# Superjie13/StereoTracking

Measured on AMD Instinct MI355X. Metric: stereo frame-pairs/sec @1280x720 D=192, higher is better.
Workload: dtype f32; 1 GPU; configs[1]: batch=8 synthetic 1280x720 stereo pairs per GPU, D=192, full YOLOX-s two-branch backbone+PAFPN+head, cost volume at 1/4 res (48 levels) + 2 3x3 aggregation convs + soft-argmin, decode+NMS, per-box depth; global_batch=8, inflight_contexts=4, distinct_input_batches=4, gpu_max_hw_queues=4, hip_force_dev_kernarg=1, parallelism=single process, no process group (no collective in the step), collectives_issued=0, tuning_plan=configs/tuning/mi355x.json, max_det=1000, detections_overflow=False

## Files before the change

include/stereotrack.h:

```cpp
#ifndef STEREOTRACK_H_
#define STEREOTRACK_H_

#include <stddef.h>
#include <stdint.h>

#ifdef __cplusplus
extern "C" {
#endif

#define ST_VERSION 430

enum {
  ST_OK = 0,
  ST_ERR_INVALID = -1,
  ST_ERR_HIP = -2,
  ST_ERR_STATE = -3,
  ST_ERR_WORKSPACE = -4,
  ST_ERR_NOTFOUND = -5
};

typedef void* st_stream_t;

int st_version(void);
const char* st_last_error(void);

typedef struct StConvDesc {
  const float* in_dev;
  int N, Hi, Wi, Cin, in_ld, in_off;
  const float* wgt_dev;
  const float* bias_dev;
  int Cout, KH, KW, stride, pad;
  float* out1_dev;
  int out1_ld, out1_off, split;
  float* out2_dev;
  int out2_ld, out2_off;
  float* up_dev;
  int up_ld, up_off;
  const float* res_dev;
  int res_ld, res_off;
  float post_scale;
  int act;
  const float* wgt_wino_dev;
} StConvDesc;

int st_conv2d_nhwc(const StConvDesc* d, st_stream_t stream);
int st_conv2d_nhwc_variant(const StConvDesc* d, st_stream_t stream, int variant);
size_t st_wino_packed_floats(int Cout, int Cin);
int st_wino_pack_weights(const float* packed_wgt_host, int Cout, int Cin, float* out_host);

int st_conv1x1_chain(const StConvDesc* a, const StConvDesc* b, st_stream_t stream);
size_t st_front_frag_floats(int Cout, int Cin);
int st_front_pack_frags(const float* packed_wgt_host, int Cout, int Cin, float* out_host);
int st_conv3x3s2_csp_front(const StConvDesc* a, const StConvDesc* ms, const StConvDesc* c1, const float* frag_ms_dev,
                           const float* frag_c1_dev, st_stream_t stream);
size_t st_csp_tail_frag_floats(void);
int st_csp_tail_pack_frags(const float* packed_wgt_host, float* out_host);
int st_conv3x3_csp_tail(const StConvDesc* conv2, const StConvDesc* fin, const float* frag_fin_dev, st_stream_t stream);
size_t st_conv_packed_floats(int Cout, int Cin, int KH, int KW);
int st_conv_pack_weights(const float* w, const float* conv_bias,
                         const float* bn_gamma, const float* bn_beta,
                         const float* bn_mean, const float* bn_var,
                         double bn_eps, int Cout, int Cin, int KH, int KW,
                         float* wgt_out, float* bias_out);

int st_focus_pack(const float* img_nchw_dev, int N, int C, int H, int W,
                  float* out_nhwc_dev, st_stream_t stream);

size_t st_stem_packed_floats(int Cout);
int st_stem_pack_weights(const float* w, const float* conv_bias,
                         const float* bn_gamma, const float* bn_beta,
                         const float* bn_mean, const float* bn_var,
                         double bn_eps, int Cout, int used_planes, float* wgt_out, float* bias_out);
int st_stem_focus_conv(const float* img_nchw_dev, int N, int H, int W, int used_planes, const float* wgt_dev,
                       const float* bias_dev, int Cout, float* out_nhwc_dev, int out_ld, int out_off,
                       int act , st_stream_t stream);
int st_stem_focus_conv_u8(const unsigned char* const* frames_u8_dev_ptrs_host, int N, int h, int w, int H, int W,
                          float pad_value, const float* wgt_dev, const float* bias_dev, int Cout, float* out_dev,
                          int out_ld, int out_off, int act, st_stream_t stream);

int st_pack_raw_inputs(const unsigned char* img_u8_dev, const unsigned short* disp_u16_dev, int N, int h, int w,
                       int H, int W, float img_pad, float* img_out_dev, float* disp_postp_out_dev,
// ... 292 lines not shown
```

stereotracking_amd/_lib.py:

```python
import ctypes as C
import os

import torch

_HERE = os.path.dirname(os.path.abspath(__file__))
LIB_PATH = os.path.join(_HERE, 'lib', 'libstereotrack_hip.so')

ST_OK = 0
_ERR_NAMES = {-1: 'ST_ERR_INVALID', -2: 'ST_ERR_HIP', -3: 'ST_ERR_STATE', -4: 'ST_ERR_WORKSPACE',
              -5: 'ST_ERR_NOTFOUND'}


class StError(RuntimeError):
    """A libstereotrack_hip call returned a non-zero status."""


class StConvDesc(C.Structure):
    _fields_ = [
        ('in_dev', C.c_void_p),
        ('N', C.c_int), ('Hi', C.c_int), ('Wi', C.c_int), ('Cin', C.c_int), ('in_ld', C.c_int), ('in_off', C.c_int),
        ('wgt_dev', C.c_void_p), ('bias_dev', C.c_void_p),
        ('Cout', C.c_int), ('KH', C.c_int), ('KW', C.c_int), ('stride', C.c_int), ('pad', C.c_int),
        ('out1_dev', C.c_void_p), ('out1_ld', C.c_int), ('out1_off', C.c_int), ('split', C.c_int),
        ('out2_dev', C.c_void_p), ('out2_ld', C.c_int), ('out2_off', C.c_int),
# ... 55 lines not shown
        ('score_thr', C.c_float), ('iou_thr', C.c_float), ('max_det', C.c_int),
        ('scale_x', C.c_float), ('scale_y', C.c_float), ('pad_left', C.c_float), ('pad_top', C.c_float),
        ('ori_w', C.c_float), ('ori_h', C.c_float), ('nms_mask_rows', C.c_int), ('num_classes', C.c_int),
        ('single_label', C.c_int),
    ]


_vp, _i, _f, _sz = C.c_void_p, C.c_int, C.c_float, C.c_size_t
_PROTOS = {
    'st_version': (C.c_int, []),
    'st_head_row_floats': (_i, [_i]),
    'st_png_unfilter': (_i, [_vp, _i, _i, _i, _vp]),
    'st_stem_focus_conv_u8': (_i, [_vp, _i, _i, _i, _i, _i, _f, _vp, _vp, _i, _vp, _i, _i, _i, _vp]),
    'st_detector_forward_raw': (_i, [_vp, _vp, _i, _i, _f, _vp, _vp, _sz, _vp, _vp]),
    'st_detector_forward_phase0_raw': (_i, [_vp, _vp, _vp, _i, _i, _f, _vp, _sz, _vp]),
    'st_pack_raw_frames': (_i, [_vp, _i, _i, _i, _i, _i, _f, _vp, _vp]),
    'st_resize_planes': (_i, [_vp, _i, _i, _i, _i, _vp, _i, _i, _i, _i, _vp]),
    'st_detector_set_split': (_i, [_vp, _i]),
    'st_split_instances_available': (_i, []),
    'st_volume_agg3d': (_i, [_vp, _vp, _i, _i, _i, _i, _vp, _f, _i, _vp]),
    'st_last_error': (C.c_char_p, []),
    'st_conv2d_nhwc': (_i, [C.POINTER(StConvDesc), _vp]),
    'st_conv2d_nhwc_variant': (_i, [C.POINTER(StConvDesc), _vp, _i]),
    'st_conv1x1_chain': (_i, [C.POINTER(StConvDesc), C.POINTER(StConvDesc), _vp]),
    'st_front_frag_floats': (_sz, [_i, _i]),
    'st_front_pack_frags': (_i, [_vp, _i, _i, _vp]),
    'st_conv3x3s2_csp_front': (_i, [C.POINTER(StConvDesc), C.POINTER(StConvDesc), C.POINTER(StConvDesc), _vp, _vp, _vp]),
    'st_csp_tail_frag_floats': (_sz, []),
    'st_csp_tail_pack_frags': (_i, [_vp, _vp]),
    'st_conv3x3_csp_tail': (_i, [C.POINTER(StConvDesc), C.POINTER(StConvDesc), _vp, _vp]),
    'st_conv_packed_floats': (_sz, [_i, _i, _i, _i]),
    'st_wino_packed_floats': (_sz, [_i, _i]),
    'st_wino_pack_weights': (_i, [_vp, _i, _i, _vp]),
    'st_conv_pack_weights': (_i, [_vp, _vp, _vp, _vp, _vp, _vp, C.c_double, _i, _i, _i, _i, _vp, _vp]),
    'st_focus_pack': (_i, [_vp, _i, _i, _i, _i, _vp, _vp]),
    'st_stem_packed_floats': (_sz, [_i]),
    'st_stem_pack_weights': (_i, [_vp, _vp, _vp, _vp, _vp, _vp, C.c_double, _i, _i, _vp, _vp]),
    'st_stem_focus_conv': (_i, [_vp, _i, _i, _i, _i, _vp, _vp, _i, _vp, _i, _i, _i, _vp]),
    'st_pack_raw_inputs': (_i, [_vp, _vp, _i, _i, _i, _i, _i, _f, _vp, _vp, _vp, _vp]),
    'st_spp_pool': (_i, [_vp, _i, _i, _i, _i, _i, _i, _vp, _i, _i, _vp]),
    'st_detector_create': (_i, [C.POINTER(StDetectorConfig), C.POINTER(_vp)]),
    'st_detector_destroy': (_i, [_vp]),
    'st_detector_num_params': (_i, [_vp]),
    'st_detector_param_info': (_i, [_vp, _i, C.c_char_p, _i, C.POINTER(C.c_int64), C.POINTER(_i)]),
    'st_detector_set_param': (_i, [_vp, C.c_char_p, _vp, C.c_int64]),
    'st_detector_finalize': (_i, [_vp]),
    'st_detector_workspace_bytes': (_sz, [_vp]),
    'st_detector_head_floats': (_sz, [_vp]),
    'st_detector_num_levels': (_i, [_vp]),
    'st_detector_level_info': (_i, [_vp, _i, C.POINTER(_i), C.POINTER(_i), C.POINTER(_i), C.POINTER(_sz)]),
    'st_detector_forward': (_i, [_vp, _vp, _vp, _vp, _sz, _vp, _vp]),
    'st_detector_forward_phase': (_i, [_vp, _i, _vp, _vp, _vp, _vp, _sz, _vp, _vp]),
    'st_detector_macs': (C.c_double, [_vp]),
    'st_detector_set_timing': (_i, [_vp, _i]),
    'st_detector_num_ops': (_i, [_vp]),
    'st_detector_op_times': (_i, [_vp, _i, _vp, _vp, _vp, _vp, _vp]),
    'st_detector_autotune': (_i, [_vp, _vp, _sz, _vp, _vp, _i]),
    'st_conv_variant_name': (C.c_char_p, [_i]),
    'st_conv_variant_signature': (C.c_char_p, [_i]),
    'st_detector_get_tuning': (_i, [_vp, _vp, _i]),
    'st_detector_set_tuning': (_i, [_vp, _vp, _i]),
    'st_detector_op_desc': (_i, [_vp, _i, C.c_char_p, _i]),
    'st_detector_tap': (_i, [_vp, C.c_char_p, _vp, C.POINTER(_vp), C.POINTER(_i), C.POINTER(_i),
                             C.POINTER(_i), C.POINTER(_i), C.POINTER(_i)]),
    'st_decode_nms_workspace_bytes': (_sz, [C.POINTER(StDecodeDesc)]),
    'st_lapjv_extended': (_i, [_vp, _i, _i, C.c_double, _vp, _vp]),
# ... 91 lines not shown
```

stereotracking_amd/csrc/conv_igemm.hip:

```cpp
#include <algorithm>

#include <type_traits>

#include "st_common.h"

namespace st {

typedef float f32x16 __attribute__((ext_vector_type(16)));
typedef float f32x4 __attribute__((ext_vector_type(4)));
typedef unsigned int u32x4 __attribute__((ext_vector_type(4)));

struct ConvKArgs {
  const float* in;
  const float* wgt;
  const float* bias;
  float* out1;
  float* out2;
  float* up;
  const float* res;
  int Hi, Wi, Cin, in_ld, in_off;
  int Ho, Wo, HoWo, Cout;
  int KH, KW, stride, pad;
  int K, Kpad, M;
  unsigned in_bytes, wgt_bytes;
// ... 656 lines not shown
  return id >= 0 && id < kNumVariants && round_up(cout, 32) % kVariants[id].bn == 0;
}
const char* conv_variant_name(int id) {
  static const char* names[] = {"128x128", "128x64w2", "128x32w2", "64x64", "64x32w2",
                                "128x64", "128x32", "64x128", "256x64", "64x64w1", "64x32w1", "32x64w1",
                                "128x128dma", "64x64dma", "64x128dma", "128x32dma", "128x64dma",
                                "128x128dmab", "64x64dmab", "256x128dma", "256x128dmab", "256x128",
                                "128x128ws", "64x64ws", "64x128ws", "128x32ws", "128x64ws", "128x128ws2",
                                "64x128ws2", "128x128ws4"};
  return id >= 0 && id < kNumVariants ? names[id] : "-";
}

const char* conv_variant_signature(int id) {
  static const char* sigs[] = {"2, 2, 2, 2, 2, 1, 0", "2, 2, 2, 1, 2, 1, 0", "2, 1, 2, 1, 2, 1, 0",
                               "1, 1, 2, 2, 2, 1, 0", "1, 1, 2, 1, 2, 1, 0", "1, 2, 4, 1, 2, 1, 0",
                               "1, 1, 4, 1, 2, 1, 0", "1, 2, 2, 2, 2, 1, 0", "2, 2, 4, 1, 2, 1, 0",
                               "2, 2, 1, 1, 1, 1, 0", "2, 1, 1, 1, 1, 1, 0", "1, 2, 1, 1, 1, 1, 0",
                               "2, 2, 2, 2, 2, 1, 1", "1, 1, 2, 2, 2, 1, 1", "1, 2, 2, 2, 2, 1, 1",
                               "1, 1, 4, 1, 2, 1, 1", "1, 2, 4, 1, 2, 1, 1", "2, 2, 2, 2, 2, 0, 1",
                               "1, 1, 2, 2, 2, 0, 1", "2, 2, 4, 2, 2, 1, 1", "2, 2, 4, 2, 2, 0, 1",
                               "2, 2, 4, 2, 2, 1, 0", "ws 2, 2, 2, 2", "ws 1, 1, 2, 2", "ws 1, 2, 2, 2",
                               "ws 1, 1, 4, 1", "ws 1, 2, 4, 1", "ws 2, 2, 2, 2, 2", "ws 1, 2, 2, 2, 2",
                               "ws 2, 2, 2, 2, 4"};
  return id >= 0 && id < kNumVariants ? sigs[id] : "";
}

bool pw_conv_applicable(const StConvDesc& d);
int pw_conv_launch(const StConvDesc& d, hipStream_t stream, const StConvDesc* chain);
int pwr_conv_launch(const StConvDesc& d, hipStream_t stream, const StConvDesc* chain);
bool pwr_chain_applicable(const StConvDesc& d, const StConvDesc& c);
bool dc_conv_applicable(const StConvDesc& d);
int dc_conv_launch(const StConvDesc& d, hipStream_t stream);
bool wino_conv_applicable(const StConvDesc& d);
int wino_conv_launch(const StConvDesc& d, hipStream_t stream, bool narrow);
int wino_persist_launch(const StConvDesc& d, hipStream_t stream);

int conv2d_launch(const StConvDesc& d, hipStream_t stream, int force_variant, int* picked_variant) {
  ST_REQUIRE(d.in_dev && d.wgt_dev && d.bias_dev && d.out1_dev, "conv: null pointer");
  if (force_variant == 41) {
    if (picked_variant) *picked_variant = 41;
    return pw_conv_launch(d, stream, nullptr);
  }
  if (force_variant == 46) {
    if (picked_variant) *picked_variant = 46;
    return pwr_conv_launch(d, stream, nullptr);
  }
  if (force_variant == 42) {
    if (picked_variant) *picked_variant = 42;
    return dc_conv_launch(d, stream);
  }
  if (force_variant == 43 || force_variant == 44) {
    if (picked_variant) *picked_variant = force_variant;
    return wino_conv_launch(d, stream, force_variant == 44);
  }
#ifdef ST_ABLATION
  if (force_variant == 57) {
    if (picked_variant) *picked_variant = 57;
    return wino_persist_launch(d, stream);
  }
#endif
  ST_REQUIRE(d.Cin % 4 == 0 && d.in_ld % 4 == 0 && d.in_off % 4 == 0,
             "conv: Cin/in_ld/in_off must be multiples of 4 (got %d/%d/%d)", d.Cin, d.in_ld,
             d.in_off);
  ST_REQUIRE(d.N > 0 && d.Hi > 0 && d.Wi > 0 && d.Cout > 0 && d.KH > 0 && d.KW > 0 &&
                 d.stride > 0 && d.pad >= 0,
             "conv: bad geometry");
  ST_REQUIRE(d.in_off + d.Cin <= d.in_ld, "conv: input channel slice exceeds in_ld");
  const int Ho = (d.Hi + 2 * d.pad - d.KH) / d.stride + 1;
  const int Wo = (d.Wi + 2 * d.pad - d.KW) / d.stride + 1;
  ST_REQUIRE(Ho > 0 && Wo > 0, "conv: empty output");
  const int split = (d.out2_dev ? d.split : d.Cout);
  ST_REQUIRE(split >= 0 && split <= d.Cout, "conv: bad split");
  ST_REQUIRE(d.out1_off + split <= d.out1_ld, "conv: out1 slice exceeds out1_ld");
  if (d.out2_dev)
    ST_REQUIRE(d.out2_off + (d.Cout - split) <= d.out2_ld, "conv: out2 slice exceeds out2_ld");
  if (d.up_dev) ST_REQUIRE(d.up_off + d.Cout <= d.up_ld, "conv: up slice exceeds up_ld");
  if (d.res_dev) ST_REQUIRE(d.res_off + d.Cout <= d.res_ld, "conv: res slice exceeds res_ld");
  const long long M_ll = (long long)d.N * Ho * Wo;
  ST_REQUIRE(M_ll * (long long)std::max(std::max(d.out1_ld, d.out2_ld), d.res_dev ? d.res_ld : 1) < (1ll << 31) &&
                 (long long)d.N * d.Hi * d.Wi * d.in_ld < (1ll << 29) &&
                 d.KH * d.KW <= 32 &&
                 (!d.up_dev || 4 * M_ll * d.up_ld < (1ll << 31)),
             "conv: tensor exceeds 2^31 elements");
  ST_REQUIRE((long long)d.N * d.Hi * d.Wi < (1ll << 31) && M_ll < (1ll << 31),
             "conv: pixel count exceeds int32");

// ... 116 lines not shown
```

stereotracking_amd/csrc/detector.cpp:

```cpp
#include <algorithm>
#include <cmath>
#include <cstring>
#include <map>
#include <memory>
#include <vector>

#include "st_common.h"

namespace st {

int conv2d_launch(const StConvDesc& d, hipStream_t stream, int force_variant, int* picked_variant);
bool pw_conv_applicable(const StConvDesc& d);
bool pw_chain_applicable(const StConvDesc& d, const StConvDesc& c);
bool dc_conv_applicable(const StConvDesc& d);
bool wino_conv_applicable(const StConvDesc& d);
bool wino_shape_ok(int Cin, int Cout);
bool wino_group_applicable(const StConvDesc* d, int n);
int wino_group_launch(const StConvDesc* d, int n, hipStream_t stream);
size_t wino_packed_floats(int Cout, int Cin);
int wino_pack_weights(const float* packed, int Cout, int Cin, float* out);
int pw_conv_launch(const StConvDesc& d, hipStream_t stream, const StConvDesc* chain);
bool pwr_conv_applicable(const StConvDesc& d);
bool pwr_chain_applicable(const StConvDesc& d, const StConvDesc& c);
int pwr_conv_launch(const StConvDesc& d, hipStream_t stream, const StConvDesc* chain);
// ... 995 lines not shown
        ms = std::min(ms, t);
      }
      if (rc != ST_OK) break;
      if (best_v < 0 || ms < best * 0.97f) { best = ms; best_v = v; }
    }
    saved[oi].tuned = best_v;
  }
  det->force_variant = -1;
  det->ops = saved;
  det->timing = was_timing;
  (void)hipEventDestroy(e0);
  (void)hipEventDestroy(e1);
  return rc;
}

extern "C" int st_split_instances_available(void) {
#ifdef ST_ABLATION
  return 1;
#else
  return 0;
#endif
}

extern "C" int st_detector_set_split(StDetector* det, int allow) {
  if (!det) return set_error(ST_ERR_INVALID, "st_detector_set_split: null detector");
  if (allow != 0 && !st_split_instances_available())
    return set_error(ST_ERR_INVALID, "st_detector_set_split: the split-operand (bf16x3) instances are not part of the product "
                                     "library (parked in the tools build: make ABLATION=1, ST_LIBRARY=<that library>)");
  det->allow_split = allow == 1 ? 0x3F : (allow & 0x3F);
  return ST_OK;
}

extern "C" const char* st_conv_variant_name(int id) {
  return id == 56 ? "wino32tail" : id == 47 ? "headpred" : id == 46 ? "pwres" : id == 45 ? "front3x3s2" : id == 40 ? "stem6x6s2" : id == 41 ? "pw128" : id == 42 ? "dc4x32" : id == 43 ? "wino2x2" : id == 44 ? "wino2x2n" : id == 48 ? "wino2x2g" : id == 49 ? "wino2x2g+" : id == 50 ? "split128x128" : id == 51 ? "split64x64" : id == 52 ? "split128x64" : id == 53 ? "split128x128k16" : id == 54 ? "split64x64k16" : id == 55 ? "split128x64k16" : conv_variant_name(id);
}
extern "C" const char* st_conv_variant_signature(int id) {
  return id == 56 ? "wino_csp_tail (bottleneck conv2 + final_conv, persistent)" : id == 47 ? "head_pred" : id == 46 ? "pw_resident" : id == 45 ? "front_s2_csp" : id == 40 ? "stem_focus_conv" : id == 41 ? "pw_conv" : id == 42 ? "direct_conv3x3" : id >= 50 && id <= 55 ? "conv_split (bf16x3 operands)" : id == 43 ? "wino_conv3x3" : id == 48 ? "wino_conv3x3 grouped launch" : id == 49 ? "wino_conv3x3 grouped launch (rider: computed by the preceding op's launch)" : id == 44 ? "wino_conv3x3 narrow"
                                                              : conv_variant_signature(id);
}

extern "C" int st_detector_get_tuning(const StDetector* det, int* variants, int cap) {
  if (!det || !variants) return set_error(ST_ERR_INVALID, "st_detector_get_tuning: null argument");
  ST_REQUIRE(cap >= (int)det->ops.size(), "st_detector_get_tuning: capacity too small");
  for (size_t i = 0; i < det->ops.size(); ++i) variants[i] = det->ops[i].tuned;
  return ST_OK;
}

extern "C" int st_detector_set_tuning(StDetector* det, const int* variants, int n) {
  if (!det || !variants) return set_error(ST_ERR_INVALID, "st_detector_set_tuning: null argument");
  ST_REQUIRE(n == (int)det->ops.size(), "st_detector_set_tuning: expected %zu entries, got %d", det->ops.size(), n);
  for (int i = 0; i < n; ++i) {
    const Op& o = det->ops[i];
    if (variants[i] < 0 || o.type != Op::CONV) continue;
    if (variants[i] >= 41 && variants[i] <= 46) continue;
    if (variants[i] >= 50 && variants[i] <= 55) {
      ST_REQUIRE(round_up(det->convs[o.pc].cout, 32) % ((variants[i] - 50) % 3 == 0 ? 128 : 64) == 0,
                 "st_detector_set_tuning: split variant %d invalid for op %d", variants[i], i);
      continue;
    }
    ST_REQUIRE(conv_variant_valid(variants[i], det->convs[o.pc].cout), "st_detector_set_tuning: variant %d invalid for op %d",
               variants[i], i);
  }
  for (int i = 0; i < n; ++i)
    if (det->ops[i].type == Op::CONV) det->ops[i].tuned = variants[i];
  return ST_OK;
}

extern "C" int st_detector_op_desc(const StDetector* det, int i, char* buf, int cap) {
  if (!det || i < 0 || i >= (int)det->ops.size() || !buf || cap <= 0)
    return set_error(ST_ERR_INVALID, "st_detector_op_desc: bad argument");
// ... 37 lines not shown
```

stereotracking_amd/csrc/wino_conv.hip:

```cpp
#include <algorithm>
#include <cmath>
#include <cstdint>
#include <cstdlib>
#include <cstring>
#include <vector>

#include "st_common.h"
#include "wino_pk.h"

namespace st {
namespace {

constexpr int WN_TX = 8, WN_TY = 4;
constexpr int WN_WW = 2 * WN_TX + 2, WN_WH = 2 * WN_TY + 2;
constexpr int WN_PIX = WN_WW * WN_WH;
constexpr int WN_PIECES = (WN_PIX + 7) / 8;
constexpr int WN_WIN_FLOATS = WN_PIECES * 8 * 32;
constexpr int wn_lds_floats(int cbn) {
  return 4 * 2 * 32 * 32 * cbn > 2 * WN_WIN_FLOATS ? 4 * 2 * 32 * 32 * cbn : 2 * WN_WIN_FLOATS;
}

struct WinoArgs {
  const float* in;
  const float* wino;
// ... 198 lines not shown
#endif
}

__device__ __forceinline__ bool wn_block_of(unsigned bid, unsigned order, unsigned per_xcd, unsigned ncb, unsigned nblocks,
                                            unsigned& b) {
  if (order == 2) {
    const unsigned slot = bid >> 3;
    b = ((slot / ncb) * 8u + (bid & 7u)) * ncb + slot % ncb;
  } else if (order == 1) {
    b = (bid & 7u) * per_xcd + (bid >> 3);
  } else {
    b = bid;
  }
  return b < nblocks;
}
static unsigned wn_order() {
#ifdef ST_ABLATION
  if (const char* e = getenv("ST_WINO_ORDER")) return (unsigned)atoi(e);
#endif
  return 0u;
}
static unsigned wn_grid(long long blocks, unsigned ncb, unsigned order, unsigned* per_xcd) {
  *per_xcd = (unsigned)((blocks + 7) / 8);
  if (order == 1) return 8u * *per_xcd;
  if (order == 2) return (unsigned)((blocks / ncb + 7) / 8 * 8 * ncb);
  return (unsigned)blocks;
}

template <int CBN, int LCBN, bool RES, bool KTAIL>
__global__ __launch_bounds__(256, 2) void wino_conv3x3_kernel(const WinoArgs p) {
  unsigned b;
  if (!wn_block_of(blockIdx.x, p.order, p.per_xcd, (unsigned)p.ncb, p.nblocks, b)) return;
  wino_conv3x3_body<CBN, LCBN, RES, KTAIL>(p, (int)b);
}

constexpr int WN_GROUP_MAX = 6;
struct WinoGroupArgs {
  WinoArgs p[WN_GROUP_MAX];
  unsigned first[WN_GROUP_MAX + 1];
  int n;
};

template <int CBN, int LCBN>
__global__ __launch_bounds__(256, 2) void wino_conv3x3_group_kernel(const WinoGroupArgs g) {
  const unsigned bid = blockIdx.x;
  int k = 0;
#pragma unroll
  for (int q = 1; q < WN_GROUP_MAX; ++q) k += (q < g.n && bid >= g.first[q]) ? 1 : 0;
  unsigned b;
  if (!wn_block_of(bid - g.first[k], g.p[k].order, g.p[k].per_xcd, (unsigned)g.p[k].ncb, g.p[k].nblocks, b)) return;
  wino_conv3x3_body<CBN, LCBN, false, false>(g.p[k], (int)b);
}


#ifdef ST_ABLATION
constexpr int wnp_lds_floats() { return 2 * WN_WIN_FLOATS + 4 * 2 * 32 * 32; }

template <int CBN, int LCBN, bool RES, bool KTAIL>
__global__ __launch_bounds__(256, 2) void wino_conv3x3_persist_kernel(const WinoArgs p) {
#if defined(__HIP_DEVICE_COMPILE__)
  constexpr int WN_FRAG_FLOATS = LCBN * 64 * 4;
  constexpr int SPLIT = LCBN / CBN;
  extern __shared__ float4 wn_smem4[];
  float* smem = reinterpret_cast<float*>(wn_smem4);
  float* Rb = smem + 2 * WN_WIN_FLOATS;
  const int tid = threadIdx.x, lane = tid & 63, a = tid >> 6;
// ... 187 lines not shown
          if (RES) {
            const unsigned roff = ok ? (unsigned)((m * p.res_ld + p.res_off + co) * 4) : 0x80000000u;
            const f32x4 rv = __builtin_bit_cast(f32x4, __builtin_amdgcn_raw_buffer_load_b128(rrsrc, roff, 0, 0));
#pragma unroll
            for (int e = 0; e < 4; ++e) v[e] = (v[e] + rv[e]) * p.post_scale;
          }
          const unsigned off = ok ? (unsigned)((m * p.out_ld + p.out_off + co) * 4) : 0x80000000u;
          __builtin_amdgcn_raw_buffer_store_b128(__builtin_bit_cast(u32x4, v), orsrc, off, 0, 0);
        }
      }
      if (nb + 1 < CBN) __syncthreads();
    }
    if (!has_next) break;
    blk = nxt; cb = cbn; bx = bxn; by = byn; n = nn;
    if (p.nkc > 1) window_offsets(bx, by, n, poff);
    wbase = wbasen;
    b0 = (b0 + p.nkc) & 1;
  }
#endif
}

#endif

}

int wino_cbn(int Cout) {
  if (Cout <= 0) return 0;
  if (Cout % 64 == 0) return 2;
  if (Cout % 32 == 0) return 1;
  if (Cout > 32 && Cout < 64) return 2;
  return 0;
}
bool wino_shape_ok(int Cin, int Cout) { return Cin >= 16 && Cin % 4 == 0 && wino_cbn(Cout) != 0; }

size_t wino_packed_floats(int Cout, int Cin) {
  const int cb = 32 * wino_cbn(Cout);
  return cb ? (size_t)16 * round_up(Cout, cb) * round_up(Cin, 32) : 0;
}

int wino_pack_weights(const float* packed, int Cout, int Cin, float* out) {
  ST_REQUIRE(packed && out && wino_shape_ok(Cin, Cout), "wino_pack_weights: not a Winograd layer shape (Cin %d, Cout %d)",
             Cin, Cout);
  const int cbn = wino_cbn(Cout), CB = 32 * cbn;
  const int Kpad = round_up(9 * Cin, 32), ncb = round_up(Cout, CB) / CB, nkc = round_up(Cin, 32) / 32;
  static const double G[4][3] = {{1, 0, 0}, {0.5, 0.5, 0.5}, {0.5, -0.5, 0.5}, {0, 0, 1}};
  for (int cb = 0; cb < ncb; ++cb)
    for (int a = 0; a < 4; ++a)
      for (int kc = 0; kc < nkc; ++kc)
        for (int g = 0; g < 4; ++g)
          for (int b = 0; b < 4; ++b)
            for (int nb = 0; nb < cbn; ++nb)
              for (int l = 0; l < 64; ++l)
                for (int e = 0; e < 4; ++e) {
                  const int j = l & 31, h = l >> 5;
                  const int co = cb * CB + nb * 32 + j, ci = kc * 32 + 8 * g + 4 * h + e;
                  double u = 0.0;
                  if (co < Cout && ci < Cin)
                    for (int kh = 0; kh < 3; ++kh)
                      for (int kw = 0; kw < 3; ++kw)
                        u += G[a][kh] * (double)packed[(size_t)co * Kpad + (kh * 3 + kw) * Cin + ci] * G[b][kw];
                  out[(((((((size_t)cb * 4 + a) * nkc + kc) * 4 + g) * 4 + b) * cbn + nb) * 64 + l) * 4 + e] = (float)u;
                }
  return ST_OK;
}

bool wino_conv_applicable(const StConvDesc& d) {
  if (!d.wgt_wino_dev) return false;
  if (d.KH != 3 || d.KW != 3 || d.stride != 1 || d.pad != 1 || d.up_dev || d.out2_dev) return false;
  if (!wino_shape_ok(d.Cin, d.Cout)) return false;
  if ((d.in_ld | d.in_off | d.out1_ld | d.out1_off) & 3) return false;
  if ((reinterpret_cast<uintptr_t>(d.in_dev) | reinterpret_cast<uintptr_t>(d.out1_dev)) & 15) return false;
  if (d.res_dev && (((d.res_ld | d.res_off) & 3) || (reinterpret_cast<uintptr_t>(d.res_dev) & 15))) return false;
  if (d.Cout % 4) return false;
  const long long M = (long long)d.N * d.Hi * d.Wi, lim = 1ll << 31;
  if (M * d.in_ld * 4 >= lim || M * d.out1_ld * 4 >= lim) return false;
  if (d.res_dev && M * d.res_ld * 4 >= lim) return false;
  return true;
}

template <int CBN, int LCBN, bool RES, bool KTAIL = false>
static int wino_launch_instance(const WinoArgs& a, unsigned blocks, hipStream_t stream) {
  constexpr int lds = wn_lds_floats(CBN) * (int)sizeof(float);
  static int lds_set = 0;
  auto kern = wino_conv3x3_kernel<CBN, LCBN, RES, KTAIL>;
  ST_ENSURE_DYNAMIC_LDS(kern, lds, lds_set);
  hipLaunchKernelGGL(kern, dim3(a.grid), dim3(256), lds, stream, a);
  return ST_OK;
}

static int wino_fill_args(const StConvDesc& d, bool narrow, WinoArgs& a, long long* blocks_out) {
  ST_REQUIRE(wino_conv_applicable(d), "winograd conv: shape not supported (3x3 s1 p1, Cin % 4 == 0, Cout a multiple of 32 "
                                      "or <= 64, transformed weights required)");
  ST_REQUIRE(d.in_dev && d.bias_dev && d.out1_dev, "winograd conv: null pointer");
  ST_REQUIRE(d.in_off + d.Cin <= d.in_ld && d.out1_off + d.Cout <= d.out1_ld, "winograd conv: channel slice exceeds ld");
  if (d.res_dev) ST_REQUIRE(d.res_off + d.Cout <= d.res_ld, "winograd conv: res slice exceeds res_ld");
  const long long M = (long long)d.N * d.Hi * d.Wi;
  const int lcbn = wino_cbn(d.Cout);
  ST_REQUIRE(!narrow || (lcbn == 2 && d.Cout % 64 == 0), "winograd conv: the narrow instance needs Cout %% 64 == 0");
  const int cbn = narrow ? 1 : lcbn, CB = 32 * cbn;
  a.in = d.in_dev; a.wino = d.wgt_wino_dev; a.bias = d.bias_dev; a.out = d.out1_dev; a.res = d.res_dev;
  a.N = d.N; a.H = d.Hi; a.W = d.Wi; a.Cin = d.Cin; a.in_ld = d.in_ld; a.in_off = d.in_off; a.Cout = d.Cout;
  a.out_ld = d.out1_ld; a.out_off = d.out1_off; a.res_ld = d.res_ld; a.res_off = d.res_off;
  a.post_scale = d.res_dev ? d.post_scale : 1.0f;
  a.act = d.act;
  a.tbx = ceil_div(d.Wi, 2 * WN_TX); a.tby = ceil_div(d.Hi, 2 * WN_TY);
  a.ncb = round_up(d.Cout, CB) / CB; a.nkc = round_up(d.Cin, 32) / 32;
  a.in_bytes = (unsigned)(M * d.in_ld * 4);
  a.out_bytes = (unsigned)(M * d.out1_ld * 4);
  a.res_bytes = d.res_dev ? (unsigned)(M * d.res_ld * 4) : 0u;
  a.wino_bytes = (unsigned)(wino_packed_floats(d.Cout, d.Cin) * 4);
  a.g_last = 4 - (a.nkc * 32 - d.Cin) / 8;
  const long long blocks = (long long)d.N * a.tbx * a.tby * a.ncb;
  ST_REQUIRE(blocks + 8 < (1ll << 31), "winograd conv: grid too large");
  a.nblocks = (unsigned)blocks;
  a.order = wn_order();
  a.grid = wn_grid(blocks, (unsigned)a.ncb, a.order, &a.per_xcd);
  *blocks_out = blocks;
  return ST_OK;
}

int wino_conv_launch(const StConvDesc& d, hipStream_t stream, bool narrow) {
  WinoArgs a;
  long long blocks = 0;
  ST_CHECK(wino_fill_args(d, narrow, a, &blocks));
  const int lcbn = wino_cbn(d.Cout);
  const int cbn = narrow ? 1 : lcbn;
  const bool ktail = a.g_last < 4;
  int rc;
  if (ktail && cbn == 2 && !d.res_dev) rc = wino_launch_instance<2, 2, false, true>(a, (unsigned)blocks, stream);
  else if (ktail && cbn == 1 && lcbn == 1 && !d.res_dev) rc = wino_launch_instance<1, 1, false, true>(a, (unsigned)blocks, stream);
  else if (cbn == 2) rc = d.res_dev ? wino_launch_instance<2, 2, true>(a, (unsigned)blocks, stream)
                               : wino_launch_instance<2, 2, false>(a, (unsigned)blocks, stream);
  else if (lcbn == 2) rc = d.res_dev ? wino_launch_instance<1, 2, true>(a, (unsigned)blocks, stream)
                                     : wino_launch_instance<1, 2, false>(a, (unsigned)blocks, stream);
  else rc = d.res_dev ? wino_launch_instance<1, 1, true>(a, (unsigned)blocks, stream)
                      : wino_launch_instance<1, 1, false>(a, (unsigned)blocks, stream);
  ST_CHECK(rc);
  ST_CHECK_HIP(hipGetLastError());
  return ST_OK;
}


#ifdef ST_ABLATION
bool wino_persist_applicable(const StConvDesc& d) { return wino_conv_applicable(d) && wino_cbn(d.Cout) == 2; }

template <int CBN, int LCBN, bool RES, bool KTAIL>
static int wino_persist_instance(const WinoArgs& a, unsigned grid, hipStream_t stream) {
  constexpr int lds = wnp_lds_floats() * (int)sizeof(float);
  static int lds_set = 0;
  auto kern = wino_conv3x3_persist_kernel<CBN, LCBN, RES, KTAIL>;
  ST_ENSURE_DYNAMIC_LDS(kern, lds, lds_set);
  hipLaunchKernelGGL(kern, dim3(grid), dim3(256), lds, stream, a);
  return ST_OK;
}

int wino_persist_launch(const StConvDesc& d, hipStream_t stream) {
  ST_REQUIRE(wino_persist_applicable(d), "winograd conv (persistent): needs a Winograd layer with the 64-cout layout");
  WinoArgs a;
  long long blocks = 0;
  ST_CHECK(wino_fill_args(d, false, a, &blocks));
  static int cus = 0;
  if (cus == 0) {
// ... 58 lines not shown
```

Measured before the change: 1782 stereo frame-pairs/s.

## Add dedicated 48-wide Winograd conv kernel for 32<Cout<=48 layers

Adds a Winograd 3x3 conv kernel whose output-channel block is 48 instead of padding to 64. It uses 16x16x4 MFMAs and a separate repacked weight image appended to the Winograd weight buffer. This removes the wasted MFMA and weight-load work on the padded channels for layers with Cout 33..48, and it becomes the default path for those shapes when there is no residual. The old padded path stays reachable as test variant 58. A standalone MFMA k-order probe kernel is also added for testing.

Result: no change. 1793 stereo frame-pairs/s (median of 6 runs) (+0.6%).

```diff
diff --git a/include/stereotrack.h b/include/stereotrack.h
--- a/include/stereotrack.h
+++ b/include/stereotrack.h
@@ -47,6 +47,8 @@
 int st_conv2d_nhwc_variant(const StConvDesc* d, st_stream_t stream, int variant);
 size_t st_wino_packed_floats(int Cout, int Cin);
 int st_wino_pack_weights(const float* packed_wgt_host, int Cout, int Cin, float* out_host);
+int st_mfma_korder_probe(const float* a_dev, const float* b_dev, const float* c_dev, int K, int mode,
+                         const int* pos_host, float* out_dev, st_stream_t stream);
 
 int st_conv1x1_chain(const StConvDesc* a, const StConvDesc* b, st_stream_t stream);
 size_t st_front_frag_floats(int Cout, int Cin);
diff --git a/stereotracking_amd/_lib.py b/stereotracking_amd/_lib.py
--- a/stereotracking_amd/_lib.py
+++ b/stereotracking_amd/_lib.py
@@ -111,6 +111,7 @@
     'st_conv_packed_floats': (_sz, [_i, _i, _i, _i]),
     'st_wino_packed_floats': (_sz, [_i, _i]),
     'st_wino_pack_weights': (_i, [_vp, _i, _i, _vp]),
+    'st_mfma_korder_probe': (_i, [_vp, _vp, _vp, _i, _i, _vp, _vp, _vp]),
     'st_conv_pack_weights': (_i, [_vp, _vp, _vp, _vp, _vp, _vp, C.c_double, _i, _i, _i, _i, _vp, _vp]),
     'st_focus_pack': (_i, [_vp, _i, _i, _i, _i, _vp, _vp]),
     'st_stem_packed_floats': (_sz, [_i]),
diff --git a/stereotracking_amd/csrc/conv_igemm.hip b/stereotracking_amd/csrc/conv_igemm.hip
--- a/stereotracking_amd/csrc/conv_igemm.hip
+++ b/stereotracking_amd/csrc/conv_igemm.hip
@@ -712,7 +712,7 @@
 bool dc_conv_applicable(const StConvDesc& d);
 int dc_conv_launch(const StConvDesc& d, hipStream_t stream);
 bool wino_conv_applicable(const StConvDesc& d);
-int wino_conv_launch(const StConvDesc& d, hipStream_t stream, bool narrow);
+int wino_conv_launch(const StConvDesc& d, hipStream_t stream, bool narrow, bool padded64);
 int wino_persist_launch(const StConvDesc& d, hipStream_t stream);
 
 int conv2d_launch(const StConvDesc& d, hipStream_t stream, int force_variant, int* picked_variant) {
@@ -729,9 +729,9 @@
     if (picked_variant) *picked_variant = 42;
     return dc_conv_launch(d, stream);
   }
-  if (force_variant == 43 || force_variant == 44) {
+  if (force_variant == 43 || force_variant == 44 || force_variant == 58) {
     if (picked_variant) *picked_variant = force_variant;
-    return wino_conv_launch(d, stream, force_variant == 44);
+    return wino_conv_launch(d, stream, force_variant == 44, force_variant == 58);
   }
 #ifdef ST_ABLATION
   if (force_variant == 57) {
diff --git a/stereotracking_amd/csrc/detector.cpp b/stereotracking_amd/csrc/detector.cpp
--- a/stereotracking_amd/csrc/detector.cpp
+++ b/stereotracking_amd/csrc/detector.cpp
@@ -1051,10 +1051,10 @@
 }
 
 extern "C" const char* st_conv_variant_name(int id) {
-  return id == 56 ? "wino32tail" : id == 47 ? "headpred" : id == 46 ? "pwres" : id == 45 ? "front3x3s2" : id == 40 ? "stem6x6s2" : id == 41 ? "pw128" : id == 42 ? "dc4x32" : id == 43 ? "wino2x2" : id == 44 ? "wino2x2n" : id == 48 ? "wino2x2g" : id == 49 ? "wino2x2g+" : id == 50 ? "split128x128" : id == 51 ? "split64x64" : id == 52 ? "split128x64" : id == 53 ? "split128x128k16" : id == 54 ? "split64x64k16" : id == 55 ? "split128x64k16" : conv_variant_name(id);
+  return id == 56 ? "wino32tail" : id == 47 ? "headpred" : id == 46 ? "pwres" : id == 45 ? "front3x3s2" : id == 40 ? "stem6x6s2" : id == 41 ? "pw128" : id == 42 ? "dc4x32" : id == 43 ? "wino2x2" : id == 44 ? "wino2x2n" : id == 58 ? "wino2x2p64" : id == 48 ? "wino2x2g" : id == 49 ? "wino2x2g+" : id == 50 ? "split128x128" : id == 51 ? "split64x64" : id == 52 ? "split128x64" : id == 53 ? "split128x128k16" : id == 54 ? "split64x64k16" : id == 55 ? "split128x64k16" : conv_variant_name(id);
 }
 extern "C" const char* st_conv_variant_signature(int id) {
-  return id == 56 ? "wino_csp_tail (bottleneck conv2 + final_conv, persistent)" : id == 47 ? "head_pred" : id == 46 ? "pw_resident" : id == 45 ? "front_s2_csp" : id == 40 ? "stem_focus_conv" : id == 41 ? "pw_conv" : id == 42 ? "direct_conv3x3" : id >= 50 && id <= 55 ? "conv_split (bf16x3 operands)" : id == 43 ? "wino_conv3x3" : id == 48 ? "wino_conv3x3 grouped launch" : id == 49 ? "wino_conv3x3 grouped launch (rider: computed by the preceding op's launch)" : id == 44 ? "wino_conv3x3 narrow"
+  return id == 56 ? "wino_csp_tail (bottleneck conv2 + final_conv, persistent)" : id == 47 ? "head_pred" : id == 46 ? "pw_resident" : id == 45 ? "front_s2_csp" : id == 40 ? "stem_focus_conv" : id == 41 ? "pw_conv" : id == 42 ? "direct_conv3x3" : id >= 50 && id <= 55 ? "conv_split (bf16x3 operands)" : id == 43 ? "wino_conv3x3" : id == 48 ? "wino_conv3x3 grouped launch" : id == 49 ? "wino_conv3x3 grouped launch (rider: computed by the preceding op's launch)" : id == 44 ? "wino_conv3x3 narrow" : id == 58 ? "wino_conv3x3 (32 < Cout <= 48 on the padded block of 64: test / A-B id)"
                                                               : conv_variant_signature(id);
 }
 
diff --git a/stereotracking_amd/csrc/mfma_korder_probe.hip b/stereotracking_amd/csrc/mfma_korder_probe.hip
--- /dev/null
+++ b/stereotracking_amd/csrc/mfma_korder_probe.hip
@@ -0,0 +1,101 @@
+#include <hip/hip_runtime.h>
+
+#include "st_common.h"
+
+namespace st {
+namespace {
+
+typedef float kp_f32x4 __attribute__((ext_vector_type(4)));
+typedef float kp_f32x16 __attribute__((ext_vector_type(16)));
+
+struct KorderArgs {
+  const float* A;
+  const float* B;
+  const float* C;
+  float* out;
+  int K, mode;
+  int pos[4];
+};
+
+__global__ __launch_bounds__(64) void mfma_korder_probe_kernel(const KorderArgs p) {
+#if defined(__HIP_DEVICE_COMPILE__)
+  const int l = threadIdx.x;
+  const int G = p.K / 8;
+  if (p.mode == 0) {
+    for (int o = l; o < 32 * 32; o += 64) {
+      const int i = o >> 5, j = o & 31;
+      float acc = p.C[o];
+      for (int g = 0; g < G; ++g)
+        for (int t = 0; t < 8; ++t) {
+          const int k = 8 * g + 4 * (t & 1) + (t >> 1);
+          acc = __builtin_fmaf(p.A[i * p.K + k], p.B[k * 32 + j], acc);
+        }
+      p.out[o] = acc;
+    }
+  } else if (p.mode == 1) {
+    const int i = l & 31, h = l >> 5;
+    kp_f32x16 acc;
+#pragma unroll
+    for (int r = 0; r < 16; ++r) acc[r] = p.C[((r & 3) + 8 * (r >> 2) + 4 * h) * 32 + i];
+    for (int g = 0; g < G; ++g)
+      for (int s = 0; s < 4; ++s) {
+        const int k = 8 * g + 4 * p.pos[h] + s;
+        acc = __builtin_amdgcn_mfma_f32_32x32x2f32(p.A[i * p.K + k], p.B[k * 32 + i], acc, 0, 0, 0);
+      }
+#pragma unroll
+    for (int r = 0; r < 16; ++r) p.out[((r & 3) + 8 * (r >> 2) + 4 * h) * 32 + i] = acc[r];
+  } else {
+    const int r = l & 15, kk = l >> 4;
+    const int ps = p.pos[kk];
+    kp_f32x4 acc[2][2];
+#pragma unroll
+    for (int bi = 0; bi < 2; ++bi)
+#pragma unroll
+      for (int bj = 0; bj < 2; ++bj)
+#pragma unroll
+        for (int q = 0; q < 4; ++q) acc[bi][bj][q] = p.C[(16 * bi + 4 * kk + q) * 32 + 16 * bj + r];
+    for (int g = 0; g < G; ++g)
+      for (int e = 0; e < 2; ++e) {
+        const int k = 8 * g + 4 * (ps & 1) + (ps >> 1) + 2 * e;
+#pragma unroll
+        for (int bi = 0; bi < 2; ++bi)
+#pragma unroll
+          for (int bj = 0; bj < 2; ++bj)
+            acc[bi][bj] = __builtin_amdgcn_mfma_f32_16x16x4f32(p.A[(16 * bi + r) * p.K + k], p.B[k * 32 + 16 * bj + r],
+                                                               acc[bi][bj], 0, 0, 0);
+      }
+#pragma unroll
+    for (int bi = 0; bi < 2; ++bi)
+#pragma unroll
+      for (int bj = 0; bj < 2; ++bj)
+#pragma unroll
+        for (int q = 0; q < 4; ++q) p.out[(16 * bi + 4 * kk + q) * 32 + 16 * bj + r] = acc[bi][bj][q];
+  }
+#endif
+}
+
+}
+}
+
+extern "C" int st_mfma_korder_probe(const float* a_dev, const float* b_dev, const float* c_dev, int K, int mode,
+                                    const int* pos_host, float* out_dev, st_stream_t stream) {
+  using namespace st;
+  ST_REQUIRE(a_dev && b_dev && c_dev && out_dev && pos_host, "st_mfma_korder_probe: null pointer");
+  ST_REQUIRE(K > 0 && K % 8 == 0 && mode >= 0 && mode <= 2, "st_mfma_korder_probe: K %% 8 == 0, mode 0..2 (got %d, %d)", K,
+             mode);
+  KorderArgs p;
+  p.A = a_dev; p.B = b_dev; p.C = c_dev; p.out = out_dev; p.K = K; p.mode = mode;
+  const int n = mode == 1 ? 2 : 4;
+  unsigned seen = 0;
+  for (int k = 0; k < 4; ++k) {
+    p.pos[k] = k < n ? pos_host[k] : 0;
+    if (k < n) {
+      ST_REQUIRE(p.pos[k] >= 0 && p.pos[k] < n, "st_mfma_korder_probe: pos is not a permutation");
+      seen |= 1u << p.pos[k];
+    }
+  }
+  ST_REQUIRE(mode == 0 || seen == (1u << n) - 1u, "st_mfma_korder_probe: pos is not a permutation");
+  hipLaunchKernelGGL(mfma_korder_probe_kernel, dim3(1), dim3(64), 0, (hipStream_t)stream, p);
+  ST_CHECK_HIP(hipGetLastError());
+  return ST_OK;
+}
diff --git a/stereotracking_amd/csrc/wino_conv.hip b/stereotracking_amd/csrc/wino_conv.hip
--- a/stereotracking_amd/csrc/wino_conv.hip
+++ b/stereotracking_amd/csrc/wino_conv.hip
@@ -254,6 +254,199 @@
   unsigned b;
   if (!wn_block_of(blockIdx.x, p.order, p.per_xcd, (unsigned)p.ncb, p.nblocks, b)) return;
   wino_conv3x3_body<CBN, LCBN, RES, KTAIL>(p, (int)b);
+}
+
+constexpr int WN48_CB = 48;
+constexpr int WN48_LD = 52;
+constexpr int WN48_STEP_FLOATS = 64 * 6;
+constexpr int wn48_lds_floats() {
+  return 4 * 2 * 32 * WN48_LD > 2 * WN_WIN_FLOATS ? 4 * 2 * 32 * WN48_LD : 2 * WN_WIN_FLOATS;
+}
+constexpr size_t wn48_image_offset(int Cin) { return (size_t)16 * 64 * ((Cin + 31) / 32 * 32); }
+
+template <bool KTAIL>
+__global__ __launch_bounds__(256, 2) void wino_conv3x3_c48_kernel(const WinoArgs p) {
+  unsigned blk;
+  if (!wn_block_of(blockIdx.x, p.order, p.per_xcd, 1u, p.nblocks, blk)) return;
+#if defined(__HIP_DEVICE_COMPILE__)
+  extern __shared__ float4 wn_smem4[];
+  float* smem = reinterpret_cast<float*>(wn_smem4);
+  const int tid = threadIdx.x, lane = tid & 63, a = tid >> 6;
+  const int r = lane & 15, kk = lane >> 4;
+  const int hq = kk & 1, je = kk >> 1;
+  int b_ = (int)blk;
+  const int bx = b_ % p.tbx; b_ /= p.tbx;
+  const int by = b_ % p.tby;
+  const int n = b_ / p.tby;
+  const int wy0 = by * (2 * WN_TY) - 1, wx0 = bx * (2 * WN_TX) - 1;
+
+  const __amdgpu_buffer_rsrc_t irsrc =
+      __builtin_amdgcn_make_buffer_rsrc(const_cast<float*>(p.in), 0, (int)p.in_bytes, 0x00020000);
+  const __amdgpu_buffer_rsrc_t wrsrc =
+      __builtin_amdgcn_make_buffer_rsrc(const_cast<float*>(p.wino), 0, (int)p.wino_bytes, 0x00020000);
+  const __amdgpu_buffer_rsrc_t orsrc = __builtin_amdgcn_make_buffer_rsrc(p.out, 0, (int)p.out_bytes, 0x00020000);
+
+  constexpr int NPW = (WN_PIECES + 3) / 4;
+  unsigned poff[NPW];
+  unsigned tail_ok = 0;
+#pragma unroll
+  for (int k = 0; k < NPW; ++k) {
+    const int j = a + 4 * k;
+    const int q = 8 * j + (lane >> 3), sl = lane & 7;
+    const int wr = q / WN_WW, wc = q - wr * WN_WW;
+    const int y = wy0 + wr, x = wx0 + wc;
+    const bool ok = j < WN_PIECES && q < WN_PIX && y >= 0 && y < p.H && x >= 0 && x < p.W;
+    const int quad = sl ^ ((q >> 1) & 7);
+    poff[k] = ok ? (unsigned)((((n * p.H + y) * p.W + x) * p.in_ld + p.in_off + 4 * quad) * 4) : 0x80000000u;
+    if ((p.nkc - 1) * 32 + 4 * quad < p.Cin) tail_ok |= 1u << k;
+  }
+  auto dma_window = [&](int kc, int buf) {
+    const bool last = kc == p.nkc - 1;
+#pragma unroll
+    for (int k = 0; k < NPW; ++k) {
+      const int j = a + 4 * k;
+      const unsigned off = (last && !((tail_ok >> k) & 1u)) ? 0x80000000u : poff[k];
+      if (j < WN_PIECES)
+        __builtin_amdgcn_raw_ptr_buffer_load_lds(
+            irsrc, (__attribute__((address_space(3))) void*)(smem + buf * WN_WIN_FLOATS + j * 256), 16, off,
+            kc * 128, 0, 0);
+    }
+  };
+
+  const int r0 = a == 0 ? 0 : (a == 2 ? 2 : 1);
+  const int r1 = a == 0 ? 2 : (a == 1 ? 2 : (a == 2 ? 1 : 3));
+  const f32x2 sgn = a == 1 ? f32x2{1.0f, 1.0f} : f32x2{-1.0f, -1.0f};
+  int qoff[8], qsw[8];
+#pragma unroll
+  for (int k = 0; k < 8; ++k) {
+    const int rr = k < 4 ? r0 : r1, c = k & 3;
+    const int q = (2 * (r >> 3) + rr) * WN_WW + 2 * (r & 7) + c;
+    qoff[k] = q * 32 + je;
+    qsw[k] = (q >> 1) & 7;
+  }
+
+  const unsigned wbase = (unsigned)(wn48_image_offset(p.Cin) + (size_t)a * p.nkc * 16 * WN48_STEP_FLOATS) * 4u;
+  const unsigned wb4 = wbase + lane * 16u, wb2 = wbase + 1024u + lane * 8u;
+  const int last_step = p.nkc * 16 - 1;
+  struct Frag { f32x4 w01; f32x2 w2; };
+  auto load_frag = [&](int step, Frag& f) {
+    const int soff = (step < last_step ? step : last_step) * (WN48_STEP_FLOATS * 4);
+    f.w01 = __builtin_bit_cast(f32x4, __builtin_amdgcn_raw_buffer_load_b128(wrsrc, wb4, soff, 0));
+    f.w2 = __builtin_bit_cast(f32x2, __builtin_amdgcn_raw_buffer_load_b64(wrsrc, wb2, soff, 0));
+  };
+
+  f32x4 acc[4][2][3];
+#pragma unroll
+  for (int b = 0; b < 4; ++b)
+#pragma unroll
+    for (int th = 0; th < 2; ++th)
+#pragma unroll
+      for (int nb = 0; nb < 3; ++nb)
+#pragma unroll
+        for (int q = 0; q < 4; ++q) acc[b][th][nb][q] = 0.f;
+
+  dma_window(0, 0);
+  Frag fe, fo;
+  load_frag(0, fe);
+  asm volatile("s_waitcnt vmcnt(0)" ::: "memory");
+  __syncthreads();
+
+  for (int kc = 0; kc < p.nkc; ++kc) {
+    const int buf = kc & 1;
+    if (kc + 1 < p.nkc) dma_window(kc + 1, buf ^ 1);
+    const float* win = smem + buf * WN_WIN_FLOATS;
+    const int gn = (KTAIL && kc == p.nkc - 1) ? p.g_last : 4;
+#pragma unroll
+    for (int g = 0; g < 4; ++g) {
+      if (KTAIL && g >= gn) continue;
+      f32x4 d[8];
+#pragma unroll
+      for (int k = 0; k < 8; ++k) {
+        const float* s0 = win + qoff[k] + (((2 * g + hq) ^ qsw[k]) << 2);
+        const float* s1 = win + qoff[k] + 72 * 32 + (((2 * g + hq) ^ qsw[k] ^ 4) << 2);
+        d[k] = f32x4{s0[0], s0[2], s1[0], s1[2]};
+      }
+      f32x4 P[4], V[4];
+#pragma unroll
+      for (int c = 0; c < 4; ++c) P[c] = wn_addsgn(d[c], sgn, d[4 + c]);
+      V[0] = wn_sub_mfma(P[0], P[2]);
+      V[1] = wn_add_mfma(P[1], P[2]);
+      V[2] = wn_sub_mfma(P[2], P[1]);
+      V[3] = wn_sub_mfma(P[1], P[3]);
+#pragma unroll
+      for (int b = 0; b < 4; ++b) {
+        const int step = (kc * 4 + g) * 4 + b;
+        if (b & 1) load_frag(step + 1, fe); else load_frag(step + 1, fo);
+        const Frag& f = (b & 1) ? fo : fe;
+#pragma unroll
+        for (int e = 0; e < 2; ++e)
+#pragma unroll
+          for (int th = 0; th < 2; ++th) {
+            acc[b][th][0] = __builtin_amdgcn_mfma_f32_16x16x4f32(V[b][2 * th + e], f.w01[e], acc[b][th][0], 0, 0, 0);
+            acc[b][th][1] = __builtin_amdgcn_mfma_f32_16x16x4f32(V[b][2 * th + e], f.w01[2 + e], acc[b][th][1], 0, 0, 0);
+            acc[b][th][2] = __builtin_amdgcn_mfma_f32_16x16x4f32(V[b][2 * th + e], f.w2[e], acc[b][th][2], 0, 0, 0);
+          }
+      }
+    }
+    asm volatile("s_waitcnt vmcnt(0)" ::: "memory");
+    __syncthreads();
+  }
+
+  float* Rb = smem;
+  __builtin_amdgcn_sched_barrier(0);
+  asm volatile("s_nop 11" ::: "memory");
+  __builtin_amdgcn_sched_barrier(0);
+#pragma unroll
+  for (int th = 0; th < 2; ++th)
+#pragma unroll
+    for (int nb = 0; nb < 3; ++nb)
+#pragma unroll
+      for (int q = 0; q < 4; q += 2) {
+        const int m = 16 * th + 4 * kk + q;
+        const f32x2 a0{acc[0][th][nb][q], acc[0][th][nb][q + 1]}, a1{acc[1][th][nb][q], acc[1][th][nb][q + 1]};
+        const f32x2 a2{acc[2][th][nb][q], acc[2][th][nb][q + 1]}, a3{acc[3][th][nb][q], acc[3][th][nb][q + 1]};
+        const f32x2 R0 = wn_pk_add(wn_pk_add(a0, a1), a2);
+        const f32x2 R1 = wn_pk_sub(wn_pk_sub(a1, a2), a3);
+#pragma unroll
+        for (int e = 0; e < 2; ++e) {
+          Rb[((a * 2 + 0) * 32 + m + e) * WN48_LD + nb * 16 + r] = R0[e];
+          Rb[((a * 2 + 1) * 32 + m + e) * WN48_LD + nb * 16 + r] = R1[e];
+        }
+      }
+  __syncthreads();
+  const int c4 = (lane & 15) * 4, tsel = lane >> 4;
+  if (c4 < WN48_CB) {
+    const f32x4 bias4 = *reinterpret_cast<const f32x4*>(p.bias + c4);
+    typedef unsigned u32x4 __attribute__((ext_vector_type(4)));
+#pragma unroll
+    for (int t8 = 0; t8 < 8; t8 += 4) {
+      const int txo = t8 + tsel;
+      const int t = a * 8 + txo;
+      const int oy0 = by * (2 * WN_TY) + 2 * a, ox0 = bx * (2 * WN_TX) + 2 * txo;
+#pragma unroll
+      for (int j = 0; j < 2; ++j) {
+        const f32x4 q0 = *reinterpret_cast<const f32x4*>(Rb + ((0 * 2 + j) * 32 + t) * WN48_LD + c4);
+        const f32x4 q1 = *reinterpret_cast<const f32x4*>(Rb + ((1 * 2 + j) * 32 + t) * WN48_LD + c4);
+        const f32x4 q2 = *reinterpret_cast<const f32x4*>(Rb + ((2 * 2 + j) * 32 + t) * WN48_LD + c4);
+        const f32x4 q3 = *reinterpret_cast<const f32x4*>(Rb + ((3 * 2 + j) * 32 + t) * WN48_LD + c4);
+        const f32x4 y[2] = {wn_add(wn_add(q0, q1), q2), wn_sub(wn_sub(q1, q2), q3)};
+#pragma unroll
+        for (int ii = 0; ii < 2; ++ii) {
+          const int oy = oy0 + ii, ox = ox0 + j;
+          const bool ok = oy < p.H && ox < p.W && c4 < p.Cout;
+          const int m = (n * p.H + oy) * p.W + ox;
+          f32x4 v = wn_add(y[ii], bias4);
+          if (p.act) {
+#pragma unroll
+            for (int e = 0; e < 4; ++e) v[e] = wn_silu(v[e]);
+          }
+          const unsigned off = ok ? (unsigned)((m * p.out_ld + p.out_off + c4) * 4) : 0x80000000u;
+          __builtin_amdgcn_raw_buffer_store_b128(__builtin_bit_cast(u32x4, v), orsrc, off, 0, 0);
+        }
+      }
+    }
+  }
+#endif
 }
 
 constexpr int WN_GROUP_MAX = 6;
@@ -507,10 +700,13 @@
   return 0;
 }
 bool wino_shape_ok(int Cin, int Cout) { return Cin >= 16 && Cin % 4 == 0 && wino_cbn(Cout) != 0; }
+static bool wino_c48_shape(int Cout) { return Cout > 32 && Cout <= WN48_CB; }
 
 size_t wino_packed_floats(int Cout, int Cin) {
   const int cb = 32 * wino_cbn(Cout);
-  return cb ? (size_t)16 * round_up(Cout, cb) * round_up(Cin, 32) : 0;
+  if (!cb) return 0;
+  const size_t n = (size_t)16 * round_up(Cout, cb) * round_up(Cin, 32);
+  return wino_c48_shape(Cout) ? n + (size_t)16 * WN48_CB * round_up(Cin, 32) : n;
 }
 
 int wino_pack_weights(const float* packed, int Cout, int Cin, float* out) {
@@ -536,6 +732,22 @@
                         u += G[a][kh] * (double)packed[(size_t)co * Kpad + (kh * 3 + kw) * Cin + ci] * G[b][kw];
                   out[(((((((size_t)cb * 4 + a) * nkc + kc) * 4 + g) * 4 + b) * cbn + nb) * 64 + l) * 4 + e] = (float)u;
                 }
+  if (!wino_c48_shape(Cout)) return ST_OK;
+  float* out48 = out + wn48_image_offset(Cin);
+  for (int a = 0; a < 4; ++a)
+    for (int kc = 0; kc < nkc; ++kc)
+      for (int g = 0; g < 4; ++g)
+        for (int b = 0; b < 4; ++b) {
+          const size_t step = (((size_t)a * nkc + kc) * 4 + g) * 4 + b;
+          for (int nb = 0; nb < 3; ++nb)
+            for (int l = 0; l < 64; ++l)
+              for (int e = 0; e < 2; ++e) {
+                const int j = l & 15, kk = l >> 4;
+                const int co = 16 * nb + j, h = kk & 1, e4 = (kk >> 1) + 2 * e;
+                const float u = out[((step * 2 + (co >> 5)) * 64 + ((h << 5) | (co & 31))) * 4 + e4];
+                out48[step * WN48_STEP_FLOATS + (nb < 2 ? l * 4 + nb * 2 + e : 256 + l * 2 + e)] = u;
+              }
+        }
   return ST_OK;
 }
 
@@ -594,15 +806,29 @@
   return ST_OK;
 }
 
-int wino_conv_launch(const StConvDesc& d, hipStream_t stream, bool narrow) {
+template <bool KTAIL>
+static int wino_launch_c48(const WinoArgs& a, hipStream_t stream) {
+  constexpr int lds = wn48_lds_floats() * (int)sizeof(float);
+  static int lds_set = 0;
+  auto kern = wino_conv3x3_c48_kernel<KTAIL>;
+  ST_ENSURE_DYNAMIC_LDS(kern, lds, lds_set);
+  hipLaunchKernelGGL(kern, dim3(a.grid), dim3(256), lds, stream, a);
+  return ST_OK;
+}
+
+int wino_conv_launch(const StConvDesc& d, hipStream_t stream, bool narrow, bool padded64) {
   WinoArgs a;
   long long blocks = 0;
   ST_CHECK(wino_fill_args(d, narrow, a, &blocks));
   const int lcbn = wino_cbn(d.Cout);
   const int cbn = narrow ? 1 : lcbn;
   const bool ktail = a.g_last < 4;
+  ST_REQUIRE(!padded64 || (wino_c48_shape(d.Cout) && !narrow),
+             "winograd conv: the padded-64 test instance is for 32 < Cout <= 48 (got %d)", d.Cout);
   int rc;
-  if (ktail && cbn == 2 && !d.res_dev) rc = wino_launch_instance<2, 2, false, true>(a, (unsigned)blocks, stream);
+  if (wino_c48_shape(d.Cout) && !d.res_dev && !padded64)
+    rc = ktail ? wino_launch_c48<true>(a, stream) : wino_launch_c48<false>(a, stream);
+  else if (ktail && cbn == 2 && !d.res_dev) rc = wino_launch_instance<2, 2, false, true>(a, (unsigned)blocks, stream);
   else if (ktail && cbn == 1 && lcbn == 1 && !d.res_dev) rc = wino_launch_instance<1, 1, false, true>(a, (unsigned)blocks, stream);
   else if (cbn == 2) rc = d.res_dev ? wino_launch_instance<2, 2, true>(a, (unsigned)blocks, stream)
                                : wino_launch_instance<2, 2, false>(a, (unsigned)blocks, stream);
```
